# piotrmwojcik/GI-GS

Hardware: AMD Instinct MI355X
Metric: train-step renders/sec (fwd+bwd, G-buffer+indirect) at 800x800; PSNR vs the CPU oracle (higher is better)
Workload: dtype f32; 1 GPU; C2 (configs[1] TensoIR lego stand-in): 300k surface Gaussians, 800x800, SH deg 2, GI step=16 start=8 delta=0.0625; P=300000, N=640000, M=9, hip_graphs=on, fused_glue=on, gi_march=proj, rasterizer=whole step = 2 hand-captured hipGraphs (fwd, bwd), asynchronous binning

## Files before the change

gi-gs_amd/csrc/api.hip:

```cpp
#include <cstdarg>
#include <cstdio>
#include <cstdlib>
#include <cstring>
#include <map>
#include <algorithm>
#include <atomic>
#include <new>
#include <mutex>
#include <vector>

#include "gigs_internal.h"

namespace {

thread_local char g_err[512] = "";

int fail(int code, const char* fmt, ...) {
  va_list ap;
  va_start(ap, fmt);
  vsnprintf(g_err, sizeof(g_err), fmt, ap);
  va_end(ap);
  return code;
}

#define HIP_TRY(expr)                                                                      \
  do {                                                                                     \
    hipError_t _e = (expr);                                                                \
    if (_e != hipSuccess)                                                                  \
      return fail(GIGS_ERR_HIP, "%s failed: %s (%s:%d)", #expr, hipGetErrorString(_e), __FILE__, __LINE__); \
  } while (0)

#define STAGE_CHECK(name)                                                                  \
  do {                                                                                     \
    hipError_t _e = hipGetLastError();                                                     \
    if (_e == hipSuccess && debug) _e = hipStreamSynchronize(s);                           \
    if (_e != hipSuccess)                                                                  \
      return fail(GIGS_ERR_HIP, "stage '%s' failed: %s", name, hipGetErrorString(_e));     \
  } while (0)

std::mutex g_size_mu;
std::map<int, size_t> g_scan_sizes, g_sort_sizes;
size_t scan_size_cached(int P) {
  std::lock_guard<std::mutex> lk(g_size_mu);
  auto it = g_scan_sizes.find(P);
  if (it != g_scan_sizes.end()) return it->second;
  const size_t v = gigs::scan_temp_bytes(P);
  g_scan_sizes[P] = v;
  return v;
}
size_t sort_size_cached(int R) {
  int bucket = 1024;
  while (bucket < R) bucket <<= 1;
  std::lock_guard<std::mutex> lk(g_size_mu);
  auto it = g_sort_sizes.find(bucket);
  if (it != g_sort_sizes.end()) return it->second;
  const size_t v = std::max(gigs::sort_temp_bytes(bucket), gigs::long_space_bytes((size_t)gigs::kBinMaxTiles, (size_t)bucket));
  g_sort_sizes[bucket] = v;
  return v;
}

uint32_t higher_msb(uint32_t n) {
  uint32_t msb = sizeof(n) * 4;
  uint32_t step = msb;
  while (step > 1) {
    step /= 2;
    if (n >> msb) msb += step;
    else msb -= step;
  }
  if (n >> msb) msb++;
  return msb;
}

int env_int(const char* name, int dflt) {
  const char* e = getenv(name);
  return (e && e[0]) ? atoi(e) : dflt;
}
gigs::Options options_from_env() {
  gigs::Options o;
  o.struct_bytes = (int)sizeof(gigs_options);
  const char* b = getenv("GIGS_BINNING");
  o.binning_legacy = (b && strcmp(b, "legacy") == 0) ? 1 : 0;
  o.bucket_max_mean = env_int("GIGS_BUCKET_MAX_MEAN", gigs::kBucketMaxMeanList);
  const char* ll = getenv("GIGS_LONG_LISTS");
  o.long_lists = (ll && ll[0]) ? (ll[0] == '1' ? 1 : 0) : -1;
  o.bucket_target = std::max(256, env_int("GIGS_BUCKET_TARGET", 1536));
  o.bin_bands = std::max(0, env_int("GIGS_BIN_BANDS", 0));
  o.blend_cull = env_int("GIGS_BLEND_CULL", 1) != 0;
  o.pre_bwd_sh_skip = env_int("GIGS_PRE_BWD_SH_SKIP", 1) != 0;
  o.gi_march = 4;
  if (const char* e = getenv("GIGS_GI_MARCH")) {
    if (strcmp(e, "exact") == 0) o.gi_march = 0;
  }
  o.gi_cert = env_int("GIGS_GI_CERT", 1) != 0;
  o.gi_interleave = env_int("GIGS_GI_INTERLEAVE", 1) != 0;
  o.gi_tile_log2w = env_int("GIGS_GI_TILE_LOG2W", 3);
  if (o.gi_tile_log2w < 0 || o.gi_tile_log2w > 6) o.gi_tile_log2w = 3;
  o.gi_zero_rays = env_int("GIGS_GI_ZERO_RAYS", 0) != 0;
  o.spec_max8 = env_int("GIGS_SPEC_MAX8", 128);
  o.spec_max16 = env_int("GIGS_SPEC_MAX16", 1500);
  o.shade_lds_floats = env_int("GIGS_SHADE_LDS_FLOATS", 30 * 1024);
  o.shade_bwd_blocks = std::max(0, env_int("GIGS_SHADE_BWD_BLOCKS", 0));
  o.shade_bwd_rows = env_int("GIGS_SHADE_BWD_ROWS", 0) != 0;
  o.spec_sparse = env_int("GIGS_SPEC_SPARSE", 1) != 0;
  o.spec_sparse_permille = env_int("GIGS_SPEC_SPARSE_PERMILLE", 37);
  if (o.spec_sparse_permille < 0 || o.spec_sparse_permille > 1000) o.spec_sparse_permille = 37;
  return o;
}
const gigs::Ctx& ctx_of(const gigs_ctx* c) { return c ? *reinterpret_cast<const gigs::Ctx*>(c) : gigs::default_ctx(); }

struct ProfRec { gigs::Stage stage; hipEvent_t a, b; };
std::mutex g_prof_mu;
std::atomic<bool> g_prof_on{false};
std::vector<ProfRec> g_prof_recs;
std::vector<hipEvent_t> g_prof_pool;

hipEvent_t prof_event() {
  if (!g_prof_pool.empty()) {
    hipEvent_t e = g_prof_pool.back();
    g_prof_pool.pop_back();
    return e;
  }
  hipEvent_t e;
  hipEventCreate(&e);
  return e;
}

}

namespace gigs {
StageTimer::StageTimer(Stage stage, void* stream) : s_((hipStream_t)stream), stage_(stage), on_(false) {
  if (!g_prof_on.load(std::memory_order_relaxed)) return;
  std::lock_guard<std::mutex> lk(g_prof_mu);
  if (!g_prof_on.load(std::memory_order_relaxed)) return;
  on_ = true;
  a_ = prof_event();
  b_ = prof_event();
  hipEventRecord(a_, s_);
}
StageTimer::~StageTimer() {
  if (!on_) return;
  hipEventRecord(b_, s_);
  std::lock_guard<std::mutex> lk(g_prof_mu);
  g_prof_recs.push_back({stage_, a_, b_});
}

const Options& default_options() {
  static const Options o = options_from_env();
  return o;
}
const Ctx& default_ctx() {
  static const Ctx c = {default_options(), 0u, nullptr, nullptr, 0, nullptr, nullptr};
  return c;
}
}

extern "C" {
const gigs::Options* gigs_internal_options(const gigs_ctx* ctx) { return &ctx_of(ctx).opt; }
int gigs_internal_fail(int code, const char* msg) { return fail(code, "%s", msg); }
int gigs_internal_check_launch(const char* entry) {
  const hipError_t e = hipGetLastError();
  return e == hipSuccess ? 0 : fail(GIGS_ERR_HIP, "%s: launch failed: %s", entry, hipGetErrorString(e));
}
}

extern "C" {

const char* gigs_last_error(void) { return g_err; }
const char* gigs_build_arch(void) { return "gfx950"; }

size_t gigs_required_geom(int P) {
  if (P < 0) { fail(GIGS_ERR_INVALID, "P < 0"); return 0; }
  return gigs::required_bytes<gigs::GeomState>((size_t)P, scan_size_cached(P));
}
size_t gigs_required_image(int width, int height) {
  const size_t N = (size_t)width * height;
  const size_t T = (size_t)((width + GIGS_BLOCK_X - 1) / GIGS_BLOCK_X) * ((height + GIGS_BLOCK_Y - 1) / GIGS_BLOCK_Y);
  return gigs::required_bytes<gigs::ImageState>(N, T);
}
size_t gigs_required_binning(int R) {
  if (R < 0) { fail(GIGS_ERR_INVALID, "R < 0"); return 0; }
  return gigs::required_bytes<gigs::BinningState>((size_t)R, sort_size_cached(R));
}

long long gigs_geom_offset(int P, int which) {
  char* base = nullptr;
  char* p = base;
  gigs::GeomState g = gigs::GeomState::fromChunk(p, (size_t)P, 0);
  const void* ptrs[] = {g.depths, g.pos_view, g.means2D, g.cov3D, g.conic_opacity, g.rgb,
// ... 584 lines not shown
```

gi-gs_amd/csrc/pbr.hip:

```cpp
#include <cmath>
#include <cstdlib>
#include <cstring>
#include <map>
#include <mutex>
#include <vector>

#include "gigs_common.h"
#include "pixel_ops.h"

namespace gigs {

__device__ __forceinline__ v3 safe_normalize(v3 v) {
  const float l = sqrtf(v.x * v.x + v.y * v.y + v.z * v.z);
  return l > 0.0f ? v3{v.x / l, v.y / l, v.z / l} : v3{0, 0, 0};
}
__device__ __forceinline__ v3 cube_dir_raw(float fx, float fy, int side) {
  switch (side) {
    case 0: return {1, -fy, -fx};
    case 1: return {-1, -fy, fx};
    case 2: return {fx, 1, fy};
    case 3: return {fx, -1, -fy};
    case 4: return {fx, -fy, 1};
    default: return {-fx, -fy, -1};
  }
// ... 390 lines not shown
                   "v_cmpx_le_f32_e32 vcc, 0, %[w]\n\t"
                   "v_pk_add_f32 %[a01], %[a01], %[p01]\n\t"
                   "v_pk_add_f32 %[aw2], %[aw2], %[wp]\n\t"
                   "s_mov_b64 exec, %[sv]"
                   : [a01] "+v"(acc01), [aw2] "+v"(accw2), [sv] "=&s"(saved)
                   : [w] "v"(w[u]), [p01] "v"(p01), [wp] "v"(wp)
                   : "vcc");
    }
  }
  float c0 = acc01.x, c1 = acc01.y, c2 = accw2.y, wsum = accw2.x;
  c0 = group_sum_last<kLanes>(c0); c1 = group_sum_last<kLanes>(c1); c2 = group_sum_last<kLanes>(c2);
  if (!kBackward) wsum = group_sum_last<kLanes>(wsum);
  if (g == kLanes - 1 && valid) {
    if (kBackward) {
      float* q = dst + 3 * (size_t)o;
      q[0] = c0; q[1] = c1; q[2] = c2;
    } else if (kNorm) {
      float* q = dst + 3 * (size_t)o;
      q[0] = c0 / wsum; q[1] = c1 / wsum; q[2] = c2 / wsum;
      wsum_out[o] = wsum;
    } else {
      float* q = dst + 4 * (size_t)o;
      q[0] = c0; q[1] = c1; q[2] = c2; q[3] = wsum;
    }
  }
}

template <bool kBackward, bool kNorm, int kLanes>
__global__ void __launch_bounds__(256)
specular_apply_kernel(int N, const float* __restrict__ src, const float* __restrict__ bounds,
                      const uint32_t* __restrict__ offsets, const float* __restrict__ W,
                      float* __restrict__ dst, float* __restrict__ wsum_out) {
  specular_apply_body<kBackward, kNorm, kLanes>(blockIdx.x, N, src, bounds, offsets, W, dst, wsum_out);
}

struct SpecLevel {
  int N, lanes, block_begin;
  const float* src;
  const float* bounds;
  const uint32_t* offsets;
  const float* W;
  float* dst;
  float* wsum_out;
};
struct SpecLevels { int n; SpecLevel lv[8]; };

template <bool kBackward>
__global__ void __launch_bounds__(256) specular_apply_multi_kernel(SpecLevels L) {
  int k = 0;
#pragma unroll
  for (int i = 1; i < 8; i++)
    if (i < L.n && (int)blockIdx.x >= L.lv[i].block_begin) k = i;
  const SpecLevel& v = L.lv[k];
  const int block = (int)blockIdx.x - v.block_begin;
  if (v.lanes == 8) specular_apply_body<kBackward, true, 8>(block, v.N, v.src, v.bounds, v.offsets, v.W, v.dst, v.wsum_out);
  else if (v.lanes == 16) specular_apply_body<kBackward, true, 16>(block, v.N, v.src, v.bounds, v.offsets, v.W, v.dst, v.wsum_out);
  else specular_apply_body<kBackward, true, 64>(block, v.N, v.src, v.bounds, v.offsets, v.W, v.dst, v.wsum_out);
}

static int spec_lanes_for(const Options& o, int avg_window) {
  return (avg_window > 0 && avg_window <= o.spec_max8) ? 8 : (avg_window > 0 && avg_window <= o.spec_max16) ? 16 : 64;
}

template <bool kBackward, bool kNorm>
static void launch_specular_apply(const Options& o, int res, int avg_window, const float* src, const float* bounds,
                                  const uint32_t* offsets, const float* W, float* dst, float* wsum_out, hipStream_t s) {
  const int total = 6 * res * res;
  const int max8 = o.spec_max8, max16 = o.spec_max16;
  if (avg_window > 0 && avg_window <= max8) {
    const int waves = (total + 7) / 8;
    hipLaunchKernelGGL((specular_apply_kernel<kBackward, kNorm, 8>), dim3((waves + 3) / 4), dim3(256), 0, s, res, src,
                       bounds, offsets, W, dst, wsum_out);
  } else if (avg_window > 0 && avg_window <= max16) {
    const int waves = (total + 3) / 4;
    hipLaunchKernelGGL((specular_apply_kernel<kBackward, kNorm, 16>), dim3((waves + 3) / 4), dim3(256), 0, s, res, src,
                       bounds, offsets, W, dst, wsum_out);
  } else {
    hipLaunchKernelGGL((specular_apply_kernel<kBackward, kNorm, 64>), dim3((total + 3) / 4), dim3(256), 0, s, res, src,
                       bounds, offsets, W, dst, wsum_out);
  }
}

struct SparseLevel {
  int total, cap, block_begin, group_begin, N;
  int vec;
  int chunks;
  int lds;
  const float* src;
  float* dst;
  const float* bounds;
  const uint32_t* offsets;
  const float* Wfwd;
  const float* wsum;
  int* list;
};
struct SparseLevels { int n; SparseLevel lv[8]; };

constexpr int kCensusPerThread = 4;

__global__ void __launch_bounds__(256) specular_census_kernel(SparseLevels L, int* __restrict__ state) {
  int k = 0;
#pragma unroll
  for (int i = 1; i < 8; i++)
    if (i < L.n && (int)blockIdx.x >= L.lv[i].block_begin) k = i;
  const SparseLevel& v = L.lv[k];
  const int lane = threadIdx.x & 63;
  const int t0 = (((int)blockIdx.x - v.block_begin) * 256 + (int)threadIdx.x) * kCensusPerThread;
  bool nz[kCensusPerThread];
  if (v.vec && t0 + kCensusPerThread <= v.total) {
    const float4* s4 = reinterpret_cast<const float4*>(v.src + 3 * (size_t)t0);
    float4* d4 = reinterpret_cast<float4*>(v.dst + 3 * (size_t)t0);
    const float4 a = s4[0], b = s4[1], c = s4[2];
    nz[0] = a.x != 0.0f || a.y != 0.0f || a.z != 0.0f;
    nz[1] = a.w != 0.0f || b.x != 0.0f || b.y != 0.0f;
    nz[2] = b.z != 0.0f || b.w != 0.0f || c.x != 0.0f;
    nz[3] = c.y != 0.0f || c.z != 0.0f || c.w != 0.0f;
    const float4 z = {0.0f, 0.0f, 0.0f, 0.0f};
    d4[0] = z; d4[1] = z; d4[2] = z;
  } else {
#pragma unroll
    for (int j = 0; j < kCensusPerThread; j++) {
      nz[j] = false;
      if (t0 + j < v.total) {
        const float* s = v.src + 3 * (size_t)(t0 + j);
        float* d = v.dst + 3 * (size_t)(t0 + j);
        nz[j] = s[0] != 0.0f || s[1] != 0.0f || s[2] != 0.0f;
        d[0] = 0.0f; d[1] = 0.0f; d[2] = 0.0f;
      }
    }
  }
  unsigned long long m[kCensusPerThread];
  int wave_total = 0;
#pragma unroll
  for (int j = 0; j < kCensusPerThread; j++) { m[j] = __ballot(nz[j]); wave_total += __popcll(m[j]); }
  __shared__ int wave_base[5];
  const int wave = threadIdx.x >> 6;
  if (lane == 0) wave_base[wave] = wave_total;
  __syncthreads();
  if (threadIdx.x == 0) {
    const int t01 = wave_base[0] + wave_base[1], t012 = t01 + wave_base[2], all = t012 + wave_base[3];
    const int first = all ? atomicAdd(state + k, all) : 0;
    wave_base[3] = first + t012; wave_base[2] = first + t01; wave_base[1] = first + wave_base[0]; wave_base[0] = first;
  }
  __syncthreads();
  if (wave_total == 0) return;
  int base = wave_base[wave];
  const unsigned long long below = (1ull << lane) - 1ull;
#pragma unroll
  for (int j = 0; j < kCensusPerThread; j++) {
    const int slot = base + __popcll(m[j] & below);
    if (nz[j] && slot < v.cap) v.list[slot] = t0 + j;
    base += __popcll(m[j]);
  }
}

constexpr int kScatterU = 2;
constexpr int kLdsTile = 32;
constexpr int kLdsParts = 8;
constexpr int kLdsWide = 16;

__global__ void __launch_bounds__(256) specular_scatter_kernel(SparseLevels L, int* __restrict__ state) {
  const int lane = threadIdx.x & 63;
  const int group = (int)blockIdx.x * 4 + ((int)threadIdx.x >> 6);
  if (blockIdx.x == 0 && threadIdx.x < 8 && (int)threadIdx.x < L.n) {
    const int c = state[threadIdx.x];
    state[8 + threadIdx.x] = c <= L.lv[threadIdx.x].cap ? 1 : 0;
    state[16 + threadIdx.x] = c;
  }
  int k = 0;
#pragma unroll
  for (int i = 1; i < 8; i++)
    if (i < L.n && group >= L.lv[i].group_begin) k = i;
  const SparseLevel& v = L.lv[k];
  const int count = state[k];
  if (count > v.cap) return;
  if (v.lds) {
    __shared__ float img[kLdsTile * kLdsTile * 3];
    const int N = v.N, nt = (N + kLdsTile - 1) / kLdsTile, bl = (group - v.group_begin) >> 2;
    const int face = bl % 6, tile = (bl / 6) % (nt * nt), part = bl / (6 * nt * nt);
    const int tx0 = (tile % nt) * kLdsTile, ty0 = (tile / nt) * kLdsTile;
    const int tx1 = min(tx0 + kLdsTile, N) - 1, ty1 = min(ty0 + kLdsTile, N) - 1;
    const int wave = (int)threadIdx.x >> 6;
    for (int i = threadIdx.x; i < kLdsTile * kLdsTile * 3; i += 256) img[i] = 0.0f;
    __syncthreads();
    const int listed = min(count, v.cap);
    for (int slot = part + kLdsParts * wave; slot < listed; slot += kLdsParts * 4) {
      const int o = __builtin_amdgcn_readfirstlane(v.list[slot]);
      const float4* b4 = reinterpret_cast<const float4*>(v.bounds + 24 * (size_t)o);
      int before = 0, xmin = 0, xmax = -1, ymin = 0, ymax = -1;
#pragma unroll
      for (int s = 0; s < 6; ++s) {
        const float4 b = b4[s];
        const int x0 = (int)b.x, x1 = (int)b.y, y0 = (int)b.z, y1 = (int)b.w;
        const int cnt = (x0 > x1 || y0 > y1) ? 0 : (x1 - x0 + 1) * (y1 - y0 + 1);
        if (s < face) before += cnt;
        if (s == face && cnt) { xmin = x0; xmax = x1; ymin = y0; ymax = y1; }
      }
      const int ix0 = max(xmin, tx0), ix1 = min(xmax, tx1), iy0 = max(ymin, ty0), iy1 = min(ymax, ty1);
      if (ix0 > ix1 || iy0 > iy1) continue;
      const int wd = xmax - xmin + 1, iw = ix1 - ix0 + 1, ni = iw * (iy1 - iy0 + 1);
      const float* W = v.Wfwd + v.offsets[6 * (size_t)o] + before;
      const float ws = v.wsum[o], inv = 1.0f / (float)iw;
      const float* g = v.src + 3 * (size_t)o;
      const float g0 = g[0], g1 = g[1], g2 = g[2];
      for (int i = lane; i < ni; i += 64) {
        const int ry = (int)(((float)i + 0.5f) * inv), y = iy0 + ry, x = ix0 + (i - ry * iw);
        const float w = W[(y - ymin) * wd + (x - xmin)];
        if (!(w >= 0.0f)) continue;
        float* t = img + 3 * ((y - ty0) * kLdsTile + (x - tx0));
        const float q = w / ws;
        const float v0 = q * g0, v1 = q * g1, v2 = q * g2;
        if (v0 != 0.0f) atomicAdd(t, v0);
        if (v1 != 0.0f) atomicAdd(t + 1, v1);
        if (v2 != 0.0f) atomicAdd(t + 2, v2);
      }
    }
    __syncthreads();
    const int row3 = 3 * (tx1 - tx0 + 1), cells = row3 * (ty1 - ty0 + 1);
    for (int i = threadIdx.x; i < cells; i += 256) {
      const int yy = i / row3, xc = i - yy * row3;
      const float val = img[3 * yy * kLdsTile + xc];
      if (val != 0.0f) atomicAdd(v.dst + 3 * ((size_t)(face * N + ty0 + yy) * N + tx0) + xc, val);
    }
    return;
  }
  const int slot = (group - v.group_begin) / v.chunks, chunk = (group - v.group_begin) % v.chunks;
  if (slot >= count || slot >= v.cap) return;
  const int o = __builtin_amdgcn_readfirstlane(v.list[slot]);
  const int N = v.N;
  int pre[7], wd[6], base[6];
  float inv[6];
  pre[0] = 0;
  const float4* b4 = reinterpret_cast<const float4*>(v.bounds + 24 * (size_t)o);
#pragma unroll
  for (int s = 0; s < 6; ++s) {
    const float4 b = b4[s];
    const int xmin = (int)b.x, xmax = (int)b.y, ymin = (int)b.z, ymax = (int)b.w;
    const bool empty = xmin > xmax || ymin > ymax;
    wd[s] = empty ? 1 : xmax - xmin + 1;
    inv[s] = 1.0f / (float)wd[s];
    pre[s + 1] = pre[s] + (empty ? 0 : wd[s] * (ymax - ymin + 1));
    base[s] = empty ? 0 : (s * N + ymin) * N + xmin;
  }
  const int n = pre[6];
  const float* W = v.Wfwd + v.offsets[6 * (size_t)o];
  const float ws = v.wsum[o];
  const float* g = v.src + 3 * (size_t)o;
  const float g0 = g[0], g1 = g[1], g2 = g[2];
  const int step = 64 * v.chunks;
  int from[3];
  float gch[3];
#pragma unroll
  for (int j = 0; j < 3; j++) {
    const int D = 64 * j + lane, ch = D % 3;
    from[j] = D / 3;
    gch[j] = ch == 0 ? g0 : ch == 1 ? g1 : g2;
  }
  const int ch0 = lane % 3;
  for (int c0 = 64 * chunk; c0 < n; c0 += step * kScatterU) {
    float w[kScatterU];
#pragma unroll
    for (int u = 0; u < kScatterU; u++) {
      const int c = c0 + u * step + lane;
      w[u] = c < n ? W[c] : -1.0f;
    }
#pragma unroll
    for (int u = 0; u < kScatterU; u++) {
      if (c0 + u * step >= n) break;
      const int c = c0 + u * step + lane;
      float q = -1.0f;
      int texel = 0;
      if (w[u] >= 0.0f) {
        int f = 0;
#pragma unroll
        for (int j = 1; j < 6; j++) f += c >= pre[j] ? 1 : 0;
        int f_pre = pre[0], f_wd = wd[0], f_base = base[0];
        float f_inv = inv[0];
#pragma unroll
        for (int j = 1; j < 6; j++)
          if (f == j) { f_pre = pre[j]; f_wd = wd[j]; f_base = base[j]; f_inv = inv[j]; }
        const int loc = c - f_pre;
        const int row = (int)(((float)loc + 0.5f) * f_inv);
        texel = f_base + row * N + (loc - row * f_wd);
        q = w[u] / ws;
      }
#pragma unroll
      for (int j = 0; j < 3; j++) {
        const float qq = __shfl(q, from[j]);
        const int tt = __shfl(texel, from[j]);
        const int ch = ch0 + j >= 3 ? ch0 + j - 3 : ch0 + j;
        const float val = qq * gch[j];
        if (!(qq < 0.0f) && val != 0.0f) atomicAdd(v.dst + 3 * (size_t)tt + ch, val);
      }
    }
  }
}

__global__ void __launch_bounds__(256) specular_apply_multi_bwd_sparse_kernel(SpecLevels L, int* __restrict__ state) {
  int k = 0;
#pragma unroll
  for (int i = 1; i < 8; i++)
    if (i < L.n && (int)blockIdx.x >= L.lv[i].block_begin) k = i;
  if (blockIdx.x == 0 && threadIdx.x < 8) state[threadIdx.x] = 0;
  if (state[8 + k] != 0) return;
  const SpecLevel& v = L.lv[k];
  const int block = (int)blockIdx.x - v.block_begin;
  if (v.lanes == 8) specular_apply_body<true, true, 8>(block, v.N, v.src, v.bounds, v.offsets, v.W, v.dst, v.wsum_out);
  else if (v.lanes == 16) specular_apply_body<true, true, 16>(block, v.N, v.src, v.bounds, v.offsets, v.W, v.dst, v.wsum_out);
  else specular_apply_body<true, true, 64>(block, v.N, v.src, v.bounds, v.offsets, v.W, v.dst, v.wsum_out);
}

static int spec_sparse_capacity(const Options& o, int res) {
  return (int)((long long)6 * res * res * o.spec_sparse_permille / 1000);
}

__device__ __forceinline__ int cube_face_uv(float x, float y, float z, float& u, float& v) {
  const float ax = fabsf(x), ay = fabsf(y), az = fabsf(z);
  int idx;
  float c;
  if (az > fmaxf(ax, ay)) { idx = 4; c = z; }
  else if (ay > ax) { idx = 2; c = y; y = z; }
  else { idx = 0; c = x; x = z; }
  if (c < 0.f) idx += 1;
  const float m = (1.0f / fabsf(c)) * 0.5f;
  const float m0 = (idx == 0 || idx == 5) ? -m : m;
  const float m1 = (idx != 2) ? -m : m;
  u = x * m0 + 0.5f;
  v = y * m1 + 0.5f;
  if (!isfinite(u) || !isfinite(v)) return -1;
  u = fminf(fmaxf(u, 0.f), 1.f);
  v = fminf(fmaxf(v, 0.f), 1.f);
  return idx;
}

struct Taps { int idx[4]; float w[4]; };

__device__ __forceinline__ bool cube_taps(int res, float dx, float dy, float dz, Taps& t) {
  float u, v;
  const int face = cube_face_uv(dx, dy, dz, u, v);
  if (face < 0) return false;
  const float fu = u * (float)res - 0.5f, fv = v * (float)res - 0.5f;
  const float flu = floorf(fu), flv = floorf(fv);
  const int iu0 = (int)flu, iv0 = (int)flv;
  const float tu = fu - flu, tv = fv - flv;
  float wsum = 0.0f;
  bool dropped = false;
#pragma unroll
  for (int k = 0; k < 4; k++) {
    const int ox = k & 1, oy = k >> 1;
    const int ix = iu0 + ox, iy = iv0 + oy;
    const float w = (ox ? tu : 1.0f - tu) * (oy ? tv : 1.0f - tv);
    const bool out_x = ix < 0 || ix >= res, out_y = iy < 0 || iy >= res;
    int idx;
    if (!out_x && !out_y) {
      idx = (face * res + iy) * res + ix;
    } else if (out_x && out_y) {
      idx = -1;
      dropped = true;
    } else {
      const float a = 2.0f * (((float)ix + 0.5f) / (float)res) - 1.0f;
      const float b = 2.0f * (((float)iy + 0.5f) / (float)res) - 1.0f;
      const v3 d = cube_dir_raw(a, b, face);
      float u2, v2;
      const int f2 = cube_face_uv(d.x, d.y, d.z, u2, v2);
      const int x2 = min(res - 1, max(0, (int)floorf(u2 * (float)res)));
      const int y2 = min(res - 1, max(0, (int)floorf(v2 * (float)res)));
      idx = (f2 * res + y2) * res + x2;
    }
    t.idx[k] = idx;
    t.w[k] = w;
    if (idx >= 0) wsum += w;
  }
  if (dropped) {
#pragma unroll
    for (int k = 0; k < 4; k++) t.w[k] = t.idx[k] >= 0 ? t.w[k] / wsum : 0.0f;
  }
  return true;
}

__device__ __forceinline__ bool cube_taps_precise(int res, float dx, float dy, float dz, Taps& t) {
  double x = dx, y = dy, z = dz;
  const double ax = fabs(x), ay = fabs(y), az = fabs(z);
  int face;
  double c;
  if (az > fmax(ax, ay)) { face = 4; c = z; }
  else if (ay > ax) { face = 2; c = y; y = z; }
  else { face = 0; c = x; x = z; }
  if (c < 0.0) face += 1;
  const double m = (1.0 / fabs(c)) * 0.5;
  const double m0 = (face == 0 || face == 5) ? -m : m;
  const double m1 = (face != 2) ? -m : m;
  double u = x * m0 + 0.5, v = y * m1 + 0.5;
// ... 860 lines not shown
    hipLaunchKernelGGL(gigs::specular_weights_kernel<true>, grid, dim3(256), 0, s, res, table, bounds, offsets, roughness, costheta_cutoff, weights);
  else
    hipLaunchKernelGGL(gigs::specular_weights_kernel<false>, grid, dim3(256), 0, s, res, table, bounds, offsets, roughness, costheta_cutoff, weights);
  return gigs_internal_check_launch("specular_weights");
}

int gigs_specular_weights_divide(int res, const float* bounds, const uint32_t* offsets, const float* weights,
                                 const float* texel_divisor, float* out_weights, void* stream) {
  if (res <= 0 || !bounds || !offsets || !weights || !texel_divisor || !out_weights)
    return gigs_internal_fail(GIGS_ERR_INVALID, "specular_weights_divide: bad argument");
  hipLaunchKernelGGL(gigs::specular_divide_weights_kernel, dim3((6 * res * res + 3) / 4), dim3(256), 0, (hipStream_t)stream,
                     res, bounds, offsets, weights, texel_divisor, out_weights);
  return gigs_internal_check_launch("specular_weights_divide");
}

int gigs_specular_cubemap_fwd_w(gigs_ctx* ctx, int res, const float* cubemap, const float* bounds, const uint32_t* offsets,
                                const float* weights, int avg_window, float* out, float* wsum_out, void* stream) {
  const gigs::Options& o = *gigs_internal_options(ctx);
  if (res <= 0 || !cubemap || !bounds || !offsets || !weights || !out) return gigs_internal_fail(GIGS_ERR_INVALID, "specular_cubemap_fwd_w: bad argument");
  hipStream_t s = (hipStream_t)stream;
  gigs::StageTimer timer(gigs::Stage::kCubemapFwd, stream);
  if (wsum_out)
    gigs::launch_specular_apply<false, true>(o, res, avg_window, cubemap, bounds, offsets, weights, out, wsum_out, s);
  else
    gigs::launch_specular_apply<false, false>(o, res, avg_window, cubemap, bounds, offsets, weights, out, nullptr, s);
  return gigs_internal_check_launch("specular_cubemap_fwd_w");
}

int gigs_specular_cubemap_bwd_w(gigs_ctx* ctx, int res, const float* bounds, const uint32_t* offsets, const float* weights_swapped,
                                int avg_window, const float* grad_out, int grad_is_rgb, float* grad_cubemap, void* stream) {
  const gigs::Options& o = *gigs_internal_options(ctx);
  if (res <= 0 || !bounds || !offsets || !weights_swapped || !grad_out || !grad_cubemap) return gigs_internal_fail(GIGS_ERR_INVALID, "specular_cubemap_bwd_w: bad argument");
  hipStream_t s = (hipStream_t)stream;
  gigs::StageTimer timer(gigs::Stage::kCubemapBwd, stream);
  if (grad_is_rgb)
    gigs::launch_specular_apply<true, true>(o, res, avg_window, grad_out, bounds, offsets, weights_swapped, grad_cubemap, nullptr, s);
  else
    gigs::launch_specular_apply<true, false>(o, res, avg_window, grad_out, bounds, offsets, weights_swapped, grad_cubemap, nullptr, s);
  return gigs_internal_check_launch("specular_cubemap_bwd_w");
}

static int fill_spec_level(const gigs::Options& o, const gigs_spec_level& a, gigs::SpecLevel& v, int& blocks) {
  v.N = a.res; v.lanes = gigs::spec_lanes_for(o, a.avg_window); v.block_begin = blocks;
  v.src = a.src; v.bounds = a.bounds; v.offsets = a.offsets; v.W = a.weights; v.dst = a.dst; v.wsum_out = a.wsum;
  const int total = 6 * a.res * a.res;
  const int waves = v.lanes == 64 ? total : (total + (64 / v.lanes) - 1) / (64 / v.lanes);
  blocks += (waves + 3) / 4;
  return total;
}

int gigs_specular_cubemap_multi_w(gigs_ctx* ctx, int n_levels, const gigs_spec_level* levels, int backward, void* stream) {
  const gigs::Options& o = *gigs_internal_options(ctx);
  if (n_levels <= 0 || n_levels > 8 || !levels) return gigs_internal_fail(GIGS_ERR_INVALID, "specular_cubemap_multi_w: bad level count");
  gigs::SpecLevels L;
  L.n = n_levels;
  int blocks = 0;
  for (int i = 0; i < n_levels; i++) {
    const gigs_spec_level& a = levels[i];
    if (a.res <= 0 || !a.src || !a.bounds || !a.offsets || !a.weights || !a.dst || (!backward && !a.wsum))
      return gigs_internal_fail(GIGS_ERR_INVALID, "specular_cubemap_multi_w: bad level");
    fill_spec_level(o, a, L.lv[i], blocks);
  }
  gigs::StageTimer timer(backward ? gigs::Stage::kCubemapBwd : gigs::Stage::kCubemapFwd, stream);
  if (backward) hipLaunchKernelGGL(gigs::specular_apply_multi_kernel<true>, dim3(blocks), dim3(256), 0, (hipStream_t)stream, L);
  else hipLaunchKernelGGL(gigs::specular_apply_multi_kernel<false>, dim3(blocks), dim3(256), 0, (hipStream_t)stream, L);
  return gigs_internal_check_launch("specular_cubemap_multi_w");
}

int gigs_spec_sparse_capacity(const gigs_ctx* ctx, int res) {
  if (res <= 0 || res > 4096) return gigs_internal_fail(GIGS_ERR_INVALID, "spec_sparse_capacity: bad resolution");
  return gigs::spec_sparse_capacity(*gigs_internal_options(ctx), res);
}

int gigs_specular_cubemap_multi_bwd_sparse(gigs_ctx* ctx, int n_levels, const gigs_spec_level* levels,
                                           const float* const* weights_fwd, const float* const* wsum, int* state,
                                           int* lists, void* stream) {
  const gigs::Options& o = *gigs_internal_options(ctx);
  if (!o.spec_sparse) return gigs_specular_cubemap_multi_w(ctx, n_levels, levels, 1, stream);
  if (n_levels <= 0 || n_levels > 8 || !levels || !weights_fwd || !wsum || !state || !lists)
    return gigs_internal_fail(GIGS_ERR_INVALID, "specular_cubemap_multi_bwd_sparse: bad argument");
  gigs::SpecLevels L;
  gigs::SparseLevels S;
  L.n = S.n = n_levels;
  int blocks = 0, census_blocks = 0, groups = 0;
  size_t list_begin = 0;
  for (int i = 0; i < n_levels; i++) {
    const gigs_spec_level& a = levels[i];
    if (a.res <= 0 || a.res > 4096 || !a.src || !a.bounds || !a.offsets || !a.weights || !a.dst || !weights_fwd[i] || !wsum[i])
      return gigs_internal_fail(GIGS_ERR_INVALID, "specular_cubemap_multi_bwd_sparse: bad level");
    const int total = fill_spec_level(o, a, L.lv[i], blocks);
    gigs::SparseLevel& q = S.lv[i];
    q.total = total; q.cap = gigs::spec_sparse_capacity(o, a.res); q.block_begin = census_blocks; q.group_begin = groups; q.N = a.res;
    q.vec = ((((uintptr_t)a.src) | ((uintptr_t)a.dst)) & 15) == 0;
    q.src = a.src; q.dst = a.dst; q.bounds = a.bounds; q.offsets = a.offsets; q.Wfwd = weights_fwd[i]; q.wsum = wsum[i];
    q.list = lists + list_begin;
    const int per_block = 256 * gigs::kCensusPerThread;
    census_blocks += (total + per_block - 1) / per_block;
    q.chunks = std::min(32, std::max(1, (std::max(1, a.avg_window) + 64 * 2 * gigs::kScatterU - 1) / (64 * 2 * gigs::kScatterU)));
    q.lds = (long long)a.avg_window * gigs::kLdsWide >= total;
    const int nt = (a.res + gigs::kLdsTile - 1) / gigs::kLdsTile;
    groups += q.lds ? 4 * 6 * nt * nt * gigs::kLdsParts : (q.cap * q.chunks + 3) / 4 * 4;
    list_begin += (size_t)q.cap;
  }
  hipStream_t s = (hipStream_t)stream;
  gigs::StageTimer timer(gigs::Stage::kCubemapBwd, stream);
  hipLaunchKernelGGL(gigs::specular_census_kernel, dim3(census_blocks), dim3(256), 0, s, S, state);
  hipLaunchKernelGGL(gigs::specular_scatter_kernel, dim3(std::max(1, (groups + 3) / 4)), dim3(256), 0, s, S, state);
  hipLaunchKernelGGL(gigs::specular_apply_multi_bwd_sparse_kernel, dim3(blocks), dim3(256), 0, s, L, state);
  return gigs_internal_check_launch("specular_cubemap_multi_bwd_sparse");
}

int gigs_cubemap_mip_fwd(int res_out, int channels, const float* in, float* out, void* stream) {
  if (res_out <= 0 || channels <= 0 || !in || !out) return gigs_internal_fail(GIGS_ERR_INVALID, "cubemap_mip_fwd: bad argument");
  gigs::StageTimer timer(gigs::Stage::kCubemapFwd, stream);
  hipLaunchKernelGGL(gigs::cubemap_mip_fwd_kernel, dim3((6 * res_out * res_out * channels + 255) / 256), dim3(256), 0, (hipStream_t)stream, res_out, channels, in, out);
  return gigs_internal_check_launch("cubemap_mip_fwd");
}

static int cubemap_mip_bwd(const char* entry, int res_out, const float* dout, const float* dout2, const float* add, float* din,
                           void* stream) {
  const int res = 2 * res_out;
  gigs::StageTimer timer(gigs::Stage::kCubemapBwd, stream);
  hipLaunchKernelGGL(gigs::cubemap_mip_bwd_kernel, dim3((6 * res * res + 255) / 256), dim3(256), 0, (hipStream_t)stream, res_out, dout, din, add,
                     dout2);
  return gigs_internal_check_launch(entry);
}

int gigs_cubemap_mip_bwd(int res_out, const float* dout, float* din, void* stream) {
  if (res_out <= 0 || !dout || !din) return gigs_internal_fail(GIGS_ERR_INVALID, "cubemap_mip_bwd: bad argument");
  return cubemap_mip_bwd("cubemap_mip_bwd", res_out, dout, nullptr, nullptr, din, stream);
}

int gigs_cubemap_mip_bwd_add(int res_out, const float* dout, const float* add, float* din, void* stream) {
  if (res_out <= 0 || !dout || !add || !din) return gigs_internal_fail(GIGS_ERR_INVALID, "cubemap_mip_bwd_add: bad argument");
  return cubemap_mip_bwd("cubemap_mip_bwd_add", res_out, dout, nullptr, add, din, stream);
}

int gigs_cubemap_mip_bwd_add2(int res_out, const float* dout, const float* dout2, const float* add, float* din, void* stream) {
  if (res_out <= 0 || !dout || !din) return gigs_internal_fail(GIGS_ERR_INVALID, "cubemap_mip_bwd_add2: bad argument");
  return cubemap_mip_bwd("cubemap_mip_bwd_add2", res_out, dout, dout2, add, din, stream);
}

int gigs_cube_texture_fwd(int res, const float* cubemap, int n, const float* dirs, float* out, int planar,
                          void* stream) {
  if (res <= 0 || n < 0 || !cubemap || (n > 0 && (!dirs || !out)))
    return gigs_internal_fail(GIGS_ERR_INVALID, "cube_texture_fwd: bad argument");
  if (n == 0) return 0;
  gigs::StageTimer timer(gigs::Stage::kCubemapFwd, stream);
  hipLaunchKernelGGL(gigs::cube_texture_fwd_kernel, dim3((n + 255) / 256), dim3(256), 0, (hipStream_t)stream, res,
                     cubemap, n, dirs, out, planar);
  return gigs_internal_check_launch("cube_texture_fwd");
}

int gigs_cube_texture_fwd_precise(int res, const float* cubemap, int n, const float* dirs, float* out, void* stream) {
  if (res <= 0 || n < 0 || !cubemap || (n > 0 && (!dirs || !out)))
    return gigs_internal_fail(GIGS_ERR_INVALID, "cube_texture_fwd_precise: bad argument");
  if (n == 0) return 0;
  gigs::StageTimer timer(gigs::Stage::kCubemapFwd, stream);
  hipLaunchKernelGGL(gigs::cube_texture_fwd_precise_kernel, dim3((n + 255) / 256), dim3(256), 0, (hipStream_t)stream, res,
                     cubemap, n, dirs, out);
  return gigs_internal_check_launch("cube_texture_fwd_precise");
}

int gigs_latlong_to_cubemap(int res_y, int res_x, int lat_h, int lat_w, int channels, const float* latlong, float* cubemap,
                            void* stream) {
  if (res_y <= 0 || res_x <= 0 || lat_h <= 0 || lat_w <= 0 || channels <= 0 || !latlong || !cubemap)
    return gigs_internal_fail(GIGS_ERR_INVALID, "latlong_to_cubemap: bad argument");
  const int n = 6 * res_y * res_x;
  gigs::StageTimer timer(gigs::Stage::kCubemapFwd, stream);
  hipLaunchKernelGGL(gigs::latlong_to_cubemap_kernel, dim3((n + 255) / 256), dim3(256), 0, (hipStream_t)stream, res_y, res_x,
                     lat_h, lat_w, channels, latlong, cubemap);
  return gigs_internal_check_launch("latlong_to_cubemap");
}

int gigs_latlong_to_cubemap_rot(int res_y, int res_x, int lat_h, int lat_w, int channels, const float* latlong, int n_rot,
                                const float* rotations, float* cubemap, void* stream) {
  if (n_rot < 1 || n_rot > 1024)
    return gigs_internal_fail(GIGS_ERR_INVALID, "latlong_to_cubemap_rot: n_rot outside 1..1024");
  if (res_y <= 0 || res_x <= 0 || lat_h <= 0 || lat_w <= 0 || channels <= 0 || !latlong || !rotations || !cubemap)
    return gigs_internal_fail(GIGS_ERR_INVALID, "latlong_to_cubemap_rot: bad argument");
  const int n = 6 * res_y * res_x;
  gigs::StageTimer timer(gigs::Stage::kCubemapFwd, stream);
  hipLaunchKernelGGL(gigs::latlong_to_cubemap_rot_kernel, dim3((n + 255) / 256, n_rot), dim3(256), 0, (hipStream_t)stream,
                     res_y, res_x, lat_h, lat_w, channels, latlong, rotations, cubemap);
  return gigs_internal_check_launch("latlong_to_cubemap_rot");
}

int gigs_cube_texture_bwd(int res, int n, const float* dirs, const float* g_out, float* d_cubemap, int planar,
                          void* stream) {
  if (res <= 0 || n < 0 || !d_cubemap || (n > 0 && (!dirs || !g_out)))
    return gigs_internal_fail(GIGS_ERR_INVALID, "cube_texture_bwd: bad argument");
// ... 234 lines not shown
```

Baseline: 359.8 renders/s.

## Replace LDS-atomic sparse specular scatter with tile gather and merged dense fallback

Wide sparse-backward texels are now handled by a per-16x16-tile gather. Each block stages hit records in LDS and each wave accumulates its 8x8 quad in registers, replacing the old LDS-atomic scatter. The scatter and dense-fallback kernels are merged into one launch, and the state bookkeeping moves to a tiny finish kernel. The sparse capacity threshold is raised so the sparse path is taken more often. In exchange there is more redundant bounds testing per tile, plus global atomics when the list spans several slices.

```diff
diff --git a/gi-gs_amd/csrc/api.hip b/gi-gs_amd/csrc/api.hip
--- a/gi-gs_amd/csrc/api.hip
+++ b/gi-gs_amd/csrc/api.hip
@@ -102,8 +102,8 @@
   o.shade_bwd_blocks = std::max(0, env_int("GIGS_SHADE_BWD_BLOCKS", 0));
   o.shade_bwd_rows = env_int("GIGS_SHADE_BWD_ROWS", 0) != 0;
   o.spec_sparse = env_int("GIGS_SPEC_SPARSE", 1) != 0;
-  o.spec_sparse_permille = env_int("GIGS_SPEC_SPARSE_PERMILLE", 37);
-  if (o.spec_sparse_permille < 0 || o.spec_sparse_permille > 1000) o.spec_sparse_permille = 37;
+  o.spec_sparse_permille = env_int("GIGS_SPEC_SPARSE_PERMILLE", 100);
+  if (o.spec_sparse_permille < 0 || o.spec_sparse_permille > 1000) o.spec_sparse_permille = 100;
   return o;
 }
 const gigs::Ctx& ctx_of(const gigs_ctx* c) { return c ? *reinterpret_cast<const gigs::Ctx*>(c) : gigs::default_ctx(); }
diff --git a/gi-gs_amd/csrc/pbr.hip b/gi-gs_amd/csrc/pbr.hip
--- a/gi-gs_amd/csrc/pbr.hip
+++ b/gi-gs_amd/csrc/pbr.hip
@@ -496,10 +496,11 @@
 }
 
 struct SparseLevel {
-  int total, cap, block_begin, group_begin, N;
+  int total, cap, block_begin, unit_begin, N;
   int vec;
-  int chunks;
-  int lds;
+  int narrow;
+  int nt;
+  int parts;
   const float* src;
   float* dst;
   const float* bounds;
@@ -568,77 +569,127 @@
   }
 }
 
+constexpr int kSpTile = 16;
+constexpr int kSpSlice = 256;
+constexpr int kSpU = 8;
+
+__device__ __forceinline__ void specular_tile_gather_body(const SparseLevel& v, int unit, int count) {
+  const int N = v.N, nt = v.nt, tiles = 6 * nt * nt;
+  const int part = unit / tiles, tile = unit - part * tiles;
+  const int slot = part * kSpSlice + (int)threadIdx.x, end = min(count, v.cap);
+  if (part * kSpSlice >= end) return;
+  const int face = tile / (nt * nt), tt = tile - face * nt * nt;
+  const int tx0 = (tt % nt) * kSpTile, ty0 = (tt / nt) * kSpTile;
+  const int tx1 = min(tx0 + kSpTile, N) - 1, ty1 = min(ty0 + kSpTile, N) - 1;
+  const int lane = threadIdx.x & 63, wave = (int)threadIdx.x >> 6;
+
+  __shared__ uint32_t r_base[kSpSlice];
+  __shared__ int r_wd[kSpSlice], r_x[kSpSlice], r_y[kSpSlice];
+  __shared__ float r_ws[kSpSlice], r_g0[kSpSlice], r_g1[kSpSlice], r_g2[kSpSlice];
+  __shared__ unsigned short q_rec[4][kSpSlice];
+  __shared__ int wave_cnt[4];
+
+  bool hit = false;
+  int wd = 0, px = 0, py = 0;
+  uint32_t t_base = 0;
+  float t_ws = 0.0f, t_g0 = 0.0f, t_g1 = 0.0f, t_g2 = 0.0f;
+  if (slot < end) {
+    const int o = v.list[slot];
+    const float4 b = reinterpret_cast<const float4*>(v.bounds + 24 * (size_t)o)[face];
+    const int xmin = (int)b.x, xmax = (int)b.y, ymin = (int)b.z, ymax = (int)b.w;
+    hit = xmin <= xmax && ymin <= ymax && xmin <= tx1 && xmax >= tx0 && ymin <= ty1 && ymax >= ty0;
+    if (hit) {
+      wd = xmax - xmin + 1; px = xmin | (xmax << 16); py = ymin | (ymax << 16);
+      t_base = v.offsets[6 * (size_t)o + face] - (uint32_t)(ymin * wd + xmin);
+      t_ws = v.wsum[o];
+      const float* g = v.src + 3 * (size_t)o;
+      t_g0 = g[0]; t_g1 = g[1]; t_g2 = g[2];
+    }
+  }
+  const unsigned long long hits = __ballot(hit);
+  if (lane == 0) wave_cnt[wave] = __popcll(hits);
+  __syncthreads();
+  int n_rec = 0, first = 0;
+#pragma unroll
+  for (int j = 0; j < 4; j++) {
+    if (j == wave) first = n_rec;
+    n_rec += wave_cnt[j];
+  }
+  if (n_rec == 0) return;
+  if (hit) {
+    const int j = first + __popcll(hits & ((1ull << lane) - 1ull));
+    r_base[j] = t_base; r_wd[j] = wd; r_x[j] = px; r_y[j] = py;
+    r_ws[j] = t_ws; r_g0[j] = t_g0; r_g1[j] = t_g1; r_g2[j] = t_g2;
+  }
+  __syncthreads();
+
+  const int qx0 = tx0 + (wave & 1) * 8, qy0 = ty0 + (wave >> 1) * 8;
+  if (qx0 >= N || qy0 >= N) return;
+  unsigned short* mine = q_rec[wave];
+  int n_q = 0;
+  for (int j0 = 0; j0 < n_rec; j0 += 64) {
+    const int j = j0 + lane;
+    bool t = false;
+    if (j < n_rec) {
+      const int xr = r_x[j], yr = r_y[j];
+      t = (xr & 0xffff) <= qx0 + 7 && (xr >> 16) >= qx0 && (yr & 0xffff) <= qy0 + 7 && (yr >> 16) >= qy0;
+    }
+    const unsigned long long m = __ballot(t);
+    if (t) mine[n_q + __popcll(m & ((1ull << lane) - 1ull))] = (unsigned short)j;
+    n_q += __popcll(m);
+  }
+  if (n_q == 0) return;
+  __builtin_amdgcn_fence(__ATOMIC_RELEASE, "wavefront");
+  __builtin_amdgcn_wave_barrier();
+  __builtin_amdgcn_fence(__ATOMIC_ACQUIRE, "wavefront");
+
+  const int x = qx0 + (lane & 7), y = qy0 + (lane >> 3);
+  const bool inside = x < N && y < N;
+  float a0[kSpU], a1[kSpU], a2[kSpU];
+#pragma unroll
+  for (int u = 0; u < kSpU; u++) { a0[u] = 0.0f; a1[u] = 0.0f; a2[u] = 0.0f; }
+  for (int i0 = 0; i0 < n_q; i0 += kSpU) {
+    float w[kSpU];
+    int rec[kSpU];
+#pragma unroll
+    for (int u = 0; u < kSpU; u++) {
+      const int j = mine[min(i0 + u, n_q - 1)];
+      rec[u] = j;
+      const int xr = r_x[j], yr = r_y[j];
+      const bool in = inside && i0 + u < n_q && x >= (xr & 0xffff) && x <= (xr >> 16) && y >= (yr & 0xffff) && y <= (yr >> 16);
+      const int rw = r_wd[j];
+      const uint32_t at = in ? (uint32_t)(y * rw + x) : (uint32_t)((yr & 0xffff) * rw + (xr & 0xffff));
+      const float wl = v.Wfwd[(size_t)(uint32_t)(r_base[j] + at)];
+      w[u] = in ? wl : -1.0f;
+    }
+#pragma unroll
+    for (int u = 0; u < kSpU; u++) {
+      const int j = rec[u];
+      if (w[u] >= 0.0f) {
+        const float q = w[u] / r_ws[j];
+        a0[u] += q * r_g0[j]; a1[u] += q * r_g1[j]; a2[u] += q * r_g2[j];
+      }
+    }
+  }
+#pragma unroll
+  for (int h = kSpU / 2; h > 0; h >>= 1)
+#pragma unroll
+    for (int u = 0; u < h; u++) { a0[u] += a0[u + h]; a1[u] += a1[u + h]; a2[u] += a2[u + h]; }
+  if (!inside) return;
+  float* d = v.dst + 3 * ((size_t)(face * N + y) * N + x);
+  const float val[3] = {a0[0], a1[0], a2[0]};
+#pragma unroll
+  for (int c = 0; c < 3; c++) {
+    if (!(val[c] != 0.0f)) continue;
+    if (v.parts == 1) d[c] = val[c];
+    else atomicAdd(d + c, val[c]);
+  }
+}
+
 constexpr int kScatterU = 2;
-constexpr int kLdsTile = 32;
-constexpr int kLdsParts = 8;
-constexpr int kLdsWide = 16;
-
-__global__ void __launch_bounds__(256) specular_scatter_kernel(SparseLevels L, int* __restrict__ state) {
+
+__device__ __forceinline__ void specular_scatter_body(const SparseLevel& v, int slot, int count) {
   const int lane = threadIdx.x & 63;
-  const int group = (int)blockIdx.x * 4 + ((int)threadIdx.x >> 6);
-  if (blockIdx.x == 0 && threadIdx.x < 8 && (int)threadIdx.x < L.n) {
-    const int c = state[threadIdx.x];
-    state[8 + threadIdx.x] = c <= L.lv[threadIdx.x].cap ? 1 : 0;
-    state[16 + threadIdx.x] = c;
-  }
-  int k = 0;
-#pragma unroll
-  for (int i = 1; i < 8; i++)
-    if (i < L.n && group >= L.lv[i].group_begin) k = i;
-  const SparseLevel& v = L.lv[k];
-  const int count = state[k];
-  if (count > v.cap) return;
-  if (v.lds) {
-    __shared__ float img[kLdsTile * kLdsTile * 3];
-    const int N = v.N, nt = (N + kLdsTile - 1) / kLdsTile, bl = (group - v.group_begin) >> 2;
-    const int face = bl % 6, tile = (bl / 6) % (nt * nt), part = bl / (6 * nt * nt);
-    const int tx0 = (tile % nt) * kLdsTile, ty0 = (tile / nt) * kLdsTile;
-    const int tx1 = min(tx0 + kLdsTile, N) - 1, ty1 = min(ty0 + kLdsTile, N) - 1;
-    const int wave = (int)threadIdx.x >> 6;
-    for (int i = threadIdx.x; i < kLdsTile * kLdsTile * 3; i += 256) img[i] = 0.0f;
-    __syncthreads();
-    const int listed = min(count, v.cap);
-    for (int slot = part + kLdsParts * wave; slot < listed; slot += kLdsParts * 4) {
-      const int o = __builtin_amdgcn_readfirstlane(v.list[slot]);
-      const float4* b4 = reinterpret_cast<const float4*>(v.bounds + 24 * (size_t)o);
-      int before = 0, xmin = 0, xmax = -1, ymin = 0, ymax = -1;
-#pragma unroll
-      for (int s = 0; s < 6; ++s) {
-        const float4 b = b4[s];
-        const int x0 = (int)b.x, x1 = (int)b.y, y0 = (int)b.z, y1 = (int)b.w;
-        const int cnt = (x0 > x1 || y0 > y1) ? 0 : (x1 - x0 + 1) * (y1 - y0 + 1);
-        if (s < face) before += cnt;
-        if (s == face && cnt) { xmin = x0; xmax = x1; ymin = y0; ymax = y1; }
-      }
-      const int ix0 = max(xmin, tx0), ix1 = min(xmax, tx1), iy0 = max(ymin, ty0), iy1 = min(ymax, ty1);
-      if (ix0 > ix1 || iy0 > iy1) continue;
-      const int wd = xmax - xmin + 1, iw = ix1 - ix0 + 1, ni = iw * (iy1 - iy0 + 1);
-      const float* W = v.Wfwd + v.offsets[6 * (size_t)o] + before;
-      const float ws = v.wsum[o], inv = 1.0f / (float)iw;
-      const float* g = v.src + 3 * (size_t)o;
-      const float g0 = g[0], g1 = g[1], g2 = g[2];
-      for (int i = lane; i < ni; i += 64) {
-        const int ry = (int)(((float)i + 0.5f) * inv), y = iy0 + ry, x = ix0 + (i - ry * iw);
-        const float w = W[(y - ymin) * wd + (x - xmin)];
-        if (!(w >= 0.0f)) continue;
-        float* t = img + 3 * ((y - ty0) * kLdsTile + (x - tx0));
-        const float q = w / ws;
-        const float v0 = q * g0, v1 = q * g1, v2 = q * g2;
-        if (v0 != 0.0f) atomicAdd(t, v0);
-        if (v1 != 0.0f) atomicAdd(t + 1, v1);
-        if (v2 != 0.0f) atomicAdd(t + 2, v2);
-      }
-    }
-    __syncthreads();
-    const int row3 = 3 * (tx1 - tx0 + 1), cells = row3 * (ty1 - ty0 + 1);
-    for (int i = threadIdx.x; i < cells; i += 256) {
-      const int yy = i / row3, xc = i - yy * row3;
-      const float val = img[3 * yy * kLdsTile + xc];
-      if (val != 0.0f) atomicAdd(v.dst + 3 * ((size_t)(face * N + ty0 + yy) * N + tx0) + xc, val);
-    }
-    return;
-  }
-  const int slot = (group - v.group_begin) / v.chunks, chunk = (group - v.group_begin) % v.chunks;
   if (slot >= count || slot >= v.cap) return;
   const int o = __builtin_amdgcn_readfirstlane(v.list[slot]);
   const int N = v.N;
@@ -661,7 +712,6 @@
   const float ws = v.wsum[o];
   const float* g = v.src + 3 * (size_t)o;
   const float g0 = g[0], g1 = g[1], g2 = g[2];
-  const int step = 64 * v.chunks;
   int from[3];
   float gch[3];
 #pragma unroll
@@ -671,17 +721,17 @@
     gch[j] = ch == 0 ? g0 : ch == 1 ? g1 : g2;
   }
   const int ch0 = lane % 3;
-  for (int c0 = 64 * chunk; c0 < n; c0 += step * kScatterU) {
+  for (int c0 = 0; c0 < n; c0 += 64 * kScatterU) {
     float w[kScatterU];
 #pragma unroll
     for (int u = 0; u < kScatterU; u++) {
-      const int c = c0 + u * step + lane;
+      const int c = c0 + u * 64 + lane;
       w[u] = c < n ? W[c] : -1.0f;
     }
 #pragma unroll
     for (int u = 0; u < kScatterU; u++) {
-      if (c0 + u * step >= n) break;
-      const int c = c0 + u * step + lane;
+      if (c0 + u * 64 >= n) break;
+      const int c = c0 + u * 64 + lane;
       float q = -1.0f;
       int texel = 0;
       if (w[u] >= 0.0f) {
@@ -710,18 +760,44 @@
   }
 }
 
-__global__ void __launch_bounds__(256) specular_apply_multi_bwd_sparse_kernel(SpecLevels L, int* __restrict__ state) {
+__global__ void __launch_bounds__(256)
+specular_apply_multi_bwd_sparse_kernel(SpecLevels L, SparseLevels S, int tile_units, const int* __restrict__ state) {
+  if ((int)blockIdx.x < tile_units) {
+    int k = 0;
+#pragma unroll
+    for (int i = 1; i < 8; i++)
+      if (i < S.n && (int)blockIdx.x >= S.lv[i].unit_begin) k = i;
+    const SparseLevel& v = S.lv[k];
+    const int count = state[k];
+    if (count > v.cap) return;
+    const int unit = (int)blockIdx.x - v.unit_begin;
+    if (v.narrow) specular_scatter_body(v, unit * 4 + ((int)threadIdx.x >> 6), count);
+    else specular_tile_gather_body(v, unit, count);
+    return;
+  }
+  const int gblock = (int)blockIdx.x - tile_units;
   int k = 0;
 #pragma unroll
   for (int i = 1; i < 8; i++)
-    if (i < L.n && (int)blockIdx.x >= L.lv[i].block_begin) k = i;
-  if (blockIdx.x == 0 && threadIdx.x < 8) state[threadIdx.x] = 0;
-  if (state[8 + k] != 0) return;
+    if (i < L.n && gblock >= L.lv[i].block_begin) k = i;
+  if (state[k] <= S.lv[k].cap) return;
   const SpecLevel& v = L.lv[k];
-  const int block = (int)blockIdx.x - v.block_begin;
+  const int block = gblock - v.block_begin;
   if (v.lanes == 8) specular_apply_body<true, true, 8>(block, v.N, v.src, v.bounds, v.offsets, v.W, v.dst, v.wsum_out);
   else if (v.lanes == 16) specular_apply_body<true, true, 16>(block, v.N, v.src, v.bounds, v.offsets, v.W, v.dst, v.wsum_out);
   else specular_apply_body<true, true, 64>(block, v.N, v.src, v.bounds, v.offsets, v.W, v.dst, v.wsum_out);
+}
+
+struct SparseCaps { int n; int cap[8]; };
+__global__ void __launch_bounds__(64) specular_sparse_finish_kernel(SparseCaps c, int* __restrict__ state) {
+  const int t = threadIdx.x;
+  if (t >= 8) return;
+  const int count = state[t];
+  if (t < c.n) {
+    state[8 + t] = count <= c.cap[t] ? 1 : 0;
+    state[16 + t] = count;
+  }
+  state[t] = 0;
 }
 
 static int spec_sparse_capacity(const Options& o, int res) {
@@ -1748,7 +1824,9 @@
   gigs::SpecLevels L;
   gigs::SparseLevels S;
   L.n = S.n = n_levels;
-  int blocks = 0, census_blocks = 0, groups = 0;
+  int blocks = 0, census_blocks = 0, units = 0;
+  gigs::SparseCaps caps = {};
+  caps.n = n_levels;
   size_t list_begin = 0;
   for (int i = 0; i < n_levels; i++) {
     const gigs_spec_level& a = levels[i];
@@ -1756,23 +1834,24 @@
       return gigs_internal_fail(GIGS_ERR_INVALID, "specular_cubemap_multi_bwd_sparse: bad level");
     const int total = fill_spec_level(o, a, L.lv[i], blocks);
     gigs::SparseLevel& q = S.lv[i];
-    q.total = total; q.cap = gigs::spec_sparse_capacity(o, a.res); q.block_begin = census_blocks; q.group_begin = groups; q.N = a.res;
+    q.total = total; q.cap = gigs::spec_sparse_capacity(o, a.res); q.block_begin = census_blocks; q.unit_begin = units; q.N = a.res;
     q.vec = ((((uintptr_t)a.src) | ((uintptr_t)a.dst)) & 15) == 0;
     q.src = a.src; q.dst = a.dst; q.bounds = a.bounds; q.offsets = a.offsets; q.Wfwd = weights_fwd[i]; q.wsum = wsum[i];
     q.list = lists + list_begin;
     const int per_block = 256 * gigs::kCensusPerThread;
     census_blocks += (total + per_block - 1) / per_block;
-    q.chunks = std::min(32, std::max(1, (std::max(1, a.avg_window) + 64 * 2 * gigs::kScatterU - 1) / (64 * 2 * gigs::kScatterU)));
-    q.lds = (long long)a.avg_window * gigs::kLdsWide >= total;
-    const int nt = (a.res + gigs::kLdsTile - 1) / gigs::kLdsTile;
-    groups += q.lds ? 4 * 6 * nt * nt * gigs::kLdsParts : (q.cap * q.chunks + 3) / 4 * 4;
+    q.narrow = a.avg_window <= gigs::kSpTile * gigs::kSpTile;
+    q.nt = (a.res + gigs::kSpTile - 1) / gigs::kSpTile;
+    q.parts = (q.cap + gigs::kSpSlice - 1) / gigs::kSpSlice;
+    units += q.narrow ? (q.cap + 3) / 4 : 6 * q.nt * q.nt * q.parts;
+    caps.cap[i] = q.cap;
     list_begin += (size_t)q.cap;
   }
   hipStream_t s = (hipStream_t)stream;
   gigs::StageTimer timer(gigs::Stage::kCubemapBwd, stream);
   hipLaunchKernelGGL(gigs::specular_census_kernel, dim3(census_blocks), dim3(256), 0, s, S, state);
-  hipLaunchKernelGGL(gigs::specular_scatter_kernel, dim3(std::max(1, (groups + 3) / 4)), dim3(256), 0, s, S, state);
-  hipLaunchKernelGGL(gigs::specular_apply_multi_bwd_sparse_kernel, dim3(blocks), dim3(256), 0, s, L, state);
+  hipLaunchKernelGGL(gigs::specular_apply_multi_bwd_sparse_kernel, dim3(units + blocks), dim3(256), 0, s, L, S, units, state);
+  hipLaunchKernelGGL(gigs::specular_sparse_finish_kernel, dim3(1), dim3(64), 0, s, caps, state);
   return gigs_internal_check_launch("specular_cubemap_multi_bwd_sparse");
 }
 
```

Result: faster. 372.7 renders/s, median of 6 (+3.6%).
